# rs-anderson/explicit-alignment-for-vqa-tasks

Hardware: AMD Instinct MI355X
Metric: mapper_train_samples_per_sec (higher is better)
Workload: dtype bf16; 1 GPU; cfg2: CLIP ViT-B/32 -> GPT-2-large (774M), MLP mapper, prefix 10, CC-shaped synthetic batches; per-GPU batch 64, S=42; fwd+bwd+AdamW; random-init weights; global_batch=64, seq_len=42, parallelism=dp1

## Files before the change

### explicit-alignment-for-vqa-tasks_amd/_lib.py

```python
from __future__ import annotations

import ctypes as C
import os

_HERE = os.path.dirname(os.path.abspath(__file__))
LIB_PATH = os.path.join(_HERE, "csrc", "libeavqa_hip.so")

F32, BF16 = 0, 1
ACT = {"none": 0, "tanh": 1, "relu": 2, "gelu_new": 3, "quick_gelu": 4}

i32, i64, f32, ptr = C.c_int, C.c_int64, C.c_float, C.c_void_p

SIGNATURES = {
    "eavqa_abi_version": [],
    "eavqa_strerror": [i32],
    "eavqa_check_device": [],
    "eavqa_gemm": [i32, i32, i32, i32, i32, i32, ptr, i64, ptr, i64, ptr, i64, i32, f32, ptr, i32, ptr, ptr, i64, ptr, i64, ptr],
    "eavqa_layernorm_fwd": [i32, i32, i32, i32, ptr, i64, ptr, ptr, f32, ptr, i64, ptr, ptr, ptr],
    "eavqa_layernorm_bwd": [i32, i32, i32, i32, ptr, i64, ptr, i64, ptr, ptr, ptr, ptr, ptr, i64, ptr, ptr, ptr, i64, ptr],
    "eavqa_layernorm_fwd_fp8": [i32, i32, i32, ptr, i64, ptr, ptr, f32, ptr, i64, ptr, ptr, ptr, ptr],
    "eavqa_layernorm_bwd_fp8": [i32, i32, i32, ptr, i64, ptr, i64, ptr, ptr, ptr, ptr, ptr, i64, ptr, i64, ptr, ptr],
    "eavqa_attention_fwd": [i32, i32, i32, i32, i32, i32, ptr, i64, ptr, i64, ptr, i64, ptr, i64, i64, i64, ptr, i64, ptr, i32, f32, ptr, ptr],
    "eavqa_attention_decode": [i32, i32, i32, i32, i32, ptr, i64, ptr, i64, ptr, i64, i64, ptr, ptr, i64, ptr, i64, ptr, i64, f32, ptr],
    "eavqa_attention_decode_splitk": [i32, i32, i32, i32, i32, ptr, i32, ptr, ptr, i64, ptr, i64, i64, ptr, i64, ptr, i64, f32, ptr],
    "eavqa_attention_bwd": [i32, i32, i32, i32, i32, i32, ptr, i64, ptr, i64, ptr, i64, ptr, i64, ptr, i64,
                            ptr, i64, ptr, i64, ptr, i64, ptr, ptr, i32, f32, ptr, ptr, ptr],
    "eavqa_build_prefix_rows": [i32, i32, i32, ptr, ptr, i32, i32, i32, ptr, ptr, ptr, ptr],
    "eavqa_build_fewshot_rows": [i32, i32, i32, i32, i64, ptr, ptr, i32, ptr, ptr, ptr, ptr, ptr],
    "eavqa_build_row_plan": [i32, i32, i32, ptr, ptr, ptr, ptr, ptr, ptr, ptr, ptr, ptr, ptr],
    "eavqa_copy_rows": [i32, i32, i32, i32, ptr, i64, i64, ptr, i64, i64, i64, ptr],
    "eavqa_transpose": [i32, i32, i32, ptr, i64, ptr, i64, ptr],
    "eavqa_select_rows": [i32, ptr, i32, ptr, ptr, ptr, ptr],
    "eavqa_move_rows": [i32, i32, i32, i32, ptr, i64, ptr, ptr, i64, ptr],
    "eavqa_l2_normalize_rows": [i32, i32, ptr, i64, ptr],
    "eavqa_topk_rows": [i32, i32, ptr, i64, i32, ptr, ptr, ptr],
    "eavqa_gemm_splitk_plan": [i32, i32, i32],
    "eavqa_gemm_splitk": [i32, i32, i32, i32, ptr, i64, ptr, i64, ptr, i32, ptr],
    "eavqa_splitk_finish": [i32, i32, i32, ptr, i32, ptr, i32, ptr, i64, i32, i32, ptr, i64, ptr, i64, ptr, i64, ptr],
    "eavqa_layernorm_splitk": [i32, i32, i32, ptr, i64, ptr, i32, ptr, ptr, i64, ptr, ptr, f32, ptr, i64, ptr],
    "eavqa_gemm_fp8_splitk_plan": [i32, i32, i32],
    "eavqa_gemm_fp8_splitk": [i32, i32, i32, ptr, i64, ptr, ptr, i64, f32, ptr, i32, ptr],
    "eavqa_layernorm_splitk_fp8": [i32, i32, ptr, i64, ptr, i32, ptr, ptr, i64, ptr, ptr, f32, ptr, i64, ptr, ptr],
    "eavqa_rmsnorm_splitk": [i32, i32, i32, ptr, i64, ptr, i32, ptr, i64, ptr, f32, ptr, i64, ptr],
    "eavqa_splitk_finish_gated": [i32, i32, i32, ptr, i32, i32, ptr, i64, ptr],
    "eavqa_attention_decode_splitk_rel": [i32, i32, i32, i32, i32, ptr, i32, i32, ptr, i64, ptr, i64, i64, ptr, i64, ptr, i64, f32, ptr, i64, i32, ptr],
    "eavqa_colsum": [i32, i32, i32, ptr, i64, ptr, i32, ptr],
    "eavqa_embed_assemble": [i32, i32, i32, ptr, ptr, ptr, i64, ptr, i64, ptr, i64, ptr, i64, ptr],
# ... 103 lines not shown
```

### explicit-alignment-for-vqa-tasks_amd/csrc/gemm.hip

```cpp
#include "common.h"

namespace {

struct Knobs {
    int stagger;
    int ablate;
    bool disable_fast;
    int k64_mode;
    int big_mode;
    int deep;
    int shape_mode;
    int group_n;
    bool no_row_split;
    explicit Knobs(int k = 0) : stagger(k & 15), ablate((k >> 4) & 7), disable_fast(((k >> 7) & 1) != 0), k64_mode((k >> 8) & 63),
                                big_mode((k >> 14) & 3), deep((k >> 16) & 3), shape_mode((k >> 18) & 7), group_n((k >> 21) & 15),
                                no_row_split(((k >> 25) & 1) != 0) {}
};

struct GemmParamsBase {
    const void* A; const void* B; void* C;
    const float* bias; const void* aux_in; void* aux_out; const void* residual;
    const float* row_scale;
    int M, N, K;
    int64_t lda, ldb, ldc, ld_aux, ldr;
// ... 810 lines not shown
    if (m_cnt == 0 || local >= m_cnt * n_cnt) return false;
    const int GN = p.group_n;
    if (GN <= 0) {
        tm = m_begin + local % m_cnt;
        tn = n_begin + local / m_cnt;
        return true;
    }
    const int per_group = m_cnt * GN;
    const int g = local / per_group, r = local - g * per_group;
    const int gn = min(GN, n_cnt - g * GN);
    tm = m_begin + r / gn;
    tn = n_begin + g * GN + r % gn;
    return true;
}

template <bool LNX>
__global__ __launch_bounds__(1024) void gemm_bf16_big_kernel(typename KernArg<LNX>::type pk, int gx, int gy, int tiles_m, int tiles_n) {
    const GemmParams p = widen(pk);
    extern __shared__ __attribute__((aligned(16))) char smem[];
    int tm, tn;
    if (!big_tile(p, gx, gy, tiles_m, tiles_n, tm, tn)) return;
    const int m0 = tm * GBM, n0 = tn * GBN;
    const int tid = threadIdx.x, lane = tid & 63;
    const int wave = __builtin_amdgcn_readfirstlane(tid >> 6);
    const int wm = wave >> 2, wn = wave & 3;
    const bf16_t* A = reinterpret_cast<const bf16_t*>(p.A);
    const bf16_t* B = reinterpret_cast<const bf16_t*>(p.B);

    const bf16_t* asrc[2];
    const bf16_t* bsrc[2];
#pragma unroll
    for (int i = 0; i < 2; ++i) {
        const int c = tid + 1024 * i;
        const int row = c >> 3, pc = c & 7;
        asrc[i] = A + (int64_t)min(m0 + row, p.M - 1) * p.lda + (pc ^ (row & 7)) * 8;
        bsrc[i] = B + (int64_t)min(n0 + row, p.N - 1) * p.ldb + (pc ^ (row & 7)) * 8;
// ... 104 lines not shown
    if (rem == 0 || rem > 192 || M <= GBM) return 0;
    int gx, gy;
    const int tiles_n = (N + GBN - 1) / GBN;
    const int with = (big_grid((M + GBM - 1) / GBM, tiles_n, gx, gy) + 31) / 32, without = (big_grid(M / GBM, tiles_n, gx, gy) + 31) / 32;
    return without < with ? rem : 0;
}

bool use_big(const GemmParams& p, const Knobs& kn) {
    if (p.K % GBK) return false;
    if (kn.big_mode == 1) return false;
    if (kn.big_mode == 2) return true;
    const int tiles = ((p.M + GBM - 1) / GBM) * ((p.N + GBN - 1) / GBN);
    return tiles >= 144;
}


#include "gemm_k64.hip"

inline float k64_cost(const GemmParams& p, const K64Choice& c, float* multi_round_loop = nullptr) {
    const int tiles_m = (p.M + c.bm - 1) / c.bm, tiles_n = (p.N + c.bn - 1) / c.bn;
    const GridPlan g = plan_grid(tiles_m, tiles_n, c.bm, c.bn);
    const float rounds = float((g.per_xcd + 31) / 32);
    const float loop = rounds * c.rate * (c.bm + c.bn) * (p.K / 64);
    if (multi_round_loop) *multi_round_loop = rounds > 1.f ? loop : 0.f;
    return loop + rounds * 0.1f * c.bm * c.bn + 4500.f;
}

#include "gemm_fp8.hip"

template <int MF>
// ... 311 lines not shown
                             off(residual, r0, ldr, res_es), ldr, ln ? &ln2 : nullptr, stream, 0);
        };
        int bgx, bgy;
        const int big_rounds = (big_grid((M - big_rem + GBM - 1) / GBM, (N + GBN - 1) / GBN, bgx, bgy) + 31) / 32;
        const bool many_big_tiles = big_rounds >= 4 || (big_rounds >= 2 && (M + GBM - 1) / GBM > 96);
        if (a_kc && b_kc && !kn.disable_fast && (K % 64) == 0 && kn.k64_mode != 1 && kn.shape_mode == 0 && kn.big_mode == 0 && !many_big_tiles) {
            int pick = K64_AUTO[0];
            float best_loop = 0.f;
            float best = k64_cost(p, K64_SHAPES[pick], &best_loop);
            for (int i = 1; i < N_K64_AUTO; ++i) {
                float loop;
                const float c = k64_cost(p, K64_SHAPES[K64_AUTO[i]], &loop);
                if (c < best) { best = c; pick = K64_AUTO[i]; best_loop = loop; }
            }
            best += 0.35f * best_loop;
            const float big_cost = float(big_rounds) * (float(K / 64) * (big_rounds == 1 ? 1380.f : 1530.f) + 9000.f) + 3000.f + big_split_ns;
            if (M > 64 && big_cost < best) return run_big(p);
            return K64_SHAPES[pick].launch(p, s);
        }
        if (a_kc && b_kc && !kn.disable_fast && (K % FBK) == 0 && !ln) {
            if (kn.shape_mode >= 2 && kn.shape_mode < 7) return SHAPES[kn.shape_mode - 2].launch(p, s);
            const bool big_ok = (K % GBK) == 0 && kn.big_mode != 1;
            if (big_ok && kn.big_mode == 2) return run_big(p);
            float best = tile_cost(p, 128, 128, RATE_FAST);
            int pick = -1;
            if (big_ok && use_big(p, kn)) {
                GemmParams pf = p;
                pf.M = M - big_rem;
                best = fminf(best, tile_cost(pf, 256, 256, RATE_BIG) + big_split_ns);
                pick = -2;
// ... 5 lines not shown
                }
            if (pick >= 0) return SHAPES[pick].launch(p, s);
            if (pick == -2) return run_big(p);
            return launch_fast(p, s, kn);
        }
        if (a_kc && b_kc) return launch(gemm_bf16_kernel<true, true>, p, s);
        if (a_kc && !b_kc) return launch(gemm_bf16_kernel<true, false>, p, s);
        if (!a_kc && b_kc) return launch(gemm_bf16_kernel<false, true>, p, s);
        return launch(gemm_bf16_kernel<false, false>, p, s);
    }
    if (a_kc && b_kc) return launch(gemm_f32_kernel<true, true>, p, s);
    if (a_kc && !b_kc) return launch(gemm_f32_kernel<true, false>, p, s);
    if (!a_kc && b_kc) return launch(gemm_f32_kernel<false, true>, p, s);
    return launch(gemm_f32_kernel<false, false>, p, s);
}
}

extern "C" int eavqa_gemm_ex(int dtype, int a_kc, int b_kc, int M, int N, int K,
                             const void* A, int64_t lda, const void* B, int64_t ldb,
                             void* C, int64_t ldc, int out_flags, float alpha,
                             const float* bias, int act,
                             const void* aux_in, void* aux_out, int64_t ld_aux,
                             const void* residual, int64_t ldr, void* stream, int knobs) {
    return gemm_impl(dtype, a_kc, b_kc, M, N, K, A, lda, B, ldb, C, ldc, out_flags, alpha, bias, act, aux_in, aux_out, ld_aux, residual, ldr,
                     nullptr, stream, knobs);
}

extern "C" int eavqa_gemm_ln_ex(int dtype, int a_kc, int b_kc, int M, int N, int K,
                                const void* A, int64_t lda, const void* B, int64_t ldb,
                                void* C, int64_t ldc, int out_flags, float alpha,
// ... 92 lines not shown
```

### explicit-alignment-for-vqa-tasks_amd/csrc/gemm_k64.hip

```cpp
template <int N> __device__ __forceinline__ void wait_vm() { __builtin_amdgcn_s_waitcnt(vm_only(N)); }


template <int WM, int WN, int MF, int NF, int NST_, int LW_> struct K64SGeo {
    static constexpr int NST = NST_, LW = LW_;
    static constexpr int NC = WM * WN;
    static constexpr int NT = 64 * (NC + LW);
    static constexpr int TBM = 16 * MF * WM, TBN = 16 * NF * WN;
    static constexpr int PT = (TBM + TBN) / 8;
    static constexpr int P_LO = PT / LW, P_HI = (PT + LW - 1) / LW, N_HI = PT % LW;
    static constexpr int AOPER = TBM * 128, STAGE = (TBM + TBN) * 128, RING = NST * STAGE;
    static constexpr int PITCH = TBN + 4;
    static constexpr int SP = (16 * MF * WM * PITCH * 4 <= RING) ? WM : ((16 * MF * (WM / 2) * PITCH * 4 <= RING && WM >= 2) ? WM / 2 : 1);
    static constexpr int MFC = (16 * MF * PITCH * 4 <= RING) ? MF : MF / 2;
    static constexpr int PROWS = 16 * MFC * SP;
    static constexpr int TPR = TBN / 4;
    static constexpr int RPP = NT / TPR, NPASS = (PROWS + RPP - 1) / RPP;
    static_assert((TBM + TBN) % 8 == 0 && P_LO >= 1, "stage must cut into whole pieces, at least one per loader");
    static_assert(16 * MFC * PITCH * 4 <= RING && MF % MFC == 0 && (MFC == MF || SP == 1), "C staging pass must fit the ring");
    static_assert(WM % SP == 0 && RING <= 160 * 1024 && NT <= 1024, "geometry");
    static_assert(P_HI * (NST - 1) <= 63 && NST >= 2 && NST <= 6, "vmcnt field");
};

template <class G>
__device__ __forceinline__ void k64s_loader_role(const char* A, const char* B, int64_t lda_bytes, int64_t ldb_bytes, int M, int N, int m0,
// ... 187 lines not shown
}

struct K64Choice { int bm, bn, wg_per_cu; float rate; int (*launch)(const GemmParams&, hipStream_t); };
const K64Choice K64_SHAPES[] = {
    {128, 80, 2, 1.1f, launch_k64s<4, 1, 2, 5, 3, 2>},
    {128, 80, 2, 1.1f, launch_k64s<4, 1, 2, 5, 3, 4>},
    {128, 128, 2, 1.1f, launch_k64s<2, 2, 4, 4, 2, 4>},
    {256, 128, 1, 1.97f, launch_k64s<4, 2, 4, 4, 3, 4, true>},
    {256, 160, 1, 1.93f, launch_k64s<4, 2, 4, 5, 3, 4, true>},
    {128, 80, 1, 1.56f, launch_k64s<4, 1, 2, 5, 4, 2, true>},
    {128, 96, 1, 1.1f, launch_k64s<4, 1, 2, 6, 3, 2>},
    {256, 192, 1, 1.1f, launch_k64s<4, 2, 4, 6, 2, 4>},
    {256, 256, 1, 1.1f, launch_k64s<2, 4, 8, 4, 2, 4>},
    {128, 128, 1, 1.73f, launch_k64s<2, 2, 4, 4, 3, 2, true>},
    {128, 256, 1, 1.97f, launch_k64s<2, 4, 4, 4, 3, 4, true>},
};
constexpr int N_K64 = sizeof(K64_SHAPES) / sizeof(K64_SHAPES[0]);
constexpr int K64_AUTO[] = {5, 3, 4, 9, 10};
constexpr int N_K64_AUTO = sizeof(K64_AUTO) / sizeof(K64_AUTO[0]);
```

### explicit-alignment-for-vqa-tasks_amd/csrc/seq.hip

```cpp
#include "common.h"
#include <algorithm>

namespace {

__device__ __forceinline__ int wave_iscan(int v) {
    const int lane = threadIdx.x & 63;
#pragma unroll
    for (int o = 1; o < 64; o <<= 1) {
        const int t = __shfl_up(v, o, 64);
        if (lane >= o) v += t;
    }
    return v;
}

__device__ __forceinline__ void write_positions(const int* mrow, int S, int pos_mode, int32_t* pos_row) {
    const int lane = threadIdx.x & 63;
    int carry = 0;
    for (int s0 = 0; s0 < S; s0 += 64) {
        const int s = s0 + lane;
        const int mv = (s < S) ? mrow[s] : 0;
        const int inc = wave_iscan(mv) + carry;
        if (s < S) pos_row[s] = pos_mode == 0 ? s : (inc * mv - 1 + 2);
        carry = __shfl(inc, 63, 64);
    }
// ... 297 lines not shown
        const bool keep = lab >= 0;
        const unsigned long long bal = __ballot(keep);
        if (lane == 0) wave_n[wave] = __popcll(bal);
        __syncthreads();
        int off = base;
        for (int w = 0; w < wave; ++w) off += wave_n[w];
        const int pos = off + __popcll(bal & ((1ull << lane) - 1ull));
        if (keep && pos < cap) { sel_idx[pos] = r; sel_labels[pos] = lab; }
        __syncthreads();
        if (tid == 0) { int t = 0; for (int w = 0; w < 16; ++w) t += wave_n[w]; base += t; }
        __syncthreads();
    }
    if (tid == 0 && count) count[0] = base;
}

template <typename T, bool SCATTER>
__global__ __launch_bounds__(256) void move_rows_kernel(int cols, const T* __restrict__ src, int64_t lds, const int32_t* __restrict__ idx,
                                                        T* __restrict__ dst, int64_t ldd) {
    const int i = blockIdx.x, j = idx[i];
    const T* x = src + (int64_t)(SCATTER ? i : j) * lds;
    T* y = dst + (int64_t)(SCATTER ? j : i) * ldd;
    constexpr int V = 16 / sizeof(T);
    for (int c = threadIdx.x * V; c < cols; c += 256 * V) *reinterpret_cast<uint4*>(y + c) = *reinterpret_cast<const uint4*>(x + c);
}

__global__ void zero_kernel(int n, float* out) {
    const int i = blockIdx.x * blockDim.x + threadIdx.x;
    if (i < n) out[i] = 0.f;
}

// ... 19 lines not shown
        hipLaunchKernelGGL(copy_rows_kernel<float>, dim3(B * S), dim3(256), 0, s, S, cols, (const float*)src, lds, src_batch_rows,
                           (float*)dst, ldd, dst_batch_rows, dst_row0);
    else if (dtype == EAVQA_BF16)
        hipLaunchKernelGGL(copy_rows_kernel<bf16_t>, dim3(B * S), dim3(256), 0, s, S, cols, (const bf16_t*)src, lds, src_batch_rows,
                           (bf16_t*)dst, ldd, dst_batch_rows, dst_row0);
    else return EAVQA_E_DTYPE;
    EAVQA_LAUNCH_CHECK();
    return EAVQA_OK;
}

extern "C" int eavqa_select_rows(int M, const int64_t* row_labels, int capacity, int32_t* sel_idx, int64_t* sel_labels, int32_t* count,
                                 void* stream) {
    if (M <= 0 || capacity < 0 || !row_labels || !sel_idx || !sel_labels) return EAVQA_E_ARG;
    hipLaunchKernelGGL(select_rows_kernel, dim3(1), dim3(1024), 0, reinterpret_cast<hipStream_t>(stream), M, row_labels, capacity, sel_idx,
                       sel_labels, count);
    EAVQA_LAUNCH_CHECK();
    return EAVQA_OK;
}

extern "C" int eavqa_move_rows(int dtype, int scatter, int n, int cols, const void* src, int64_t ld_src, const int32_t* idx, void* dst,
                               int64_t ld_dst, void* stream) {
    if (n < 0 || cols <= 0 || !src || !idx || !dst) return EAVQA_E_ARG;
    if (n == 0) return EAVQA_OK;
    const int vec = dtype == EAVQA_BF16 ? 8 : 4;
    if (dtype != EAVQA_BF16 && dtype != EAVQA_F32) return EAVQA_E_DTYPE;
    if (cols % vec || ld_src % vec || ld_dst % vec || !eavqa_aligned16(src) || !eavqa_aligned16(dst)) return EAVQA_E_ALIGN;
    hipStream_t s = reinterpret_cast<hipStream_t>(stream);
    if (dtype == EAVQA_BF16) {
        if (scatter) hipLaunchKernelGGL((move_rows_kernel<bf16_t, true>), dim3(n), dim3(256), 0, s, cols, (const bf16_t*)src, ld_src, idx, (bf16_t*)dst, ld_dst);
        else hipLaunchKernelGGL((move_rows_kernel<bf16_t, false>), dim3(n), dim3(256), 0, s, cols, (const bf16_t*)src, ld_src, idx, (bf16_t*)dst, ld_dst);
// ... 211 lines not shown
```

### explicit-alignment-for-vqa-tasks_amd/models/lm.py

```python
from __future__ import annotations

import json
import math
import os
from dataclasses import dataclass
from typing import Dict, Optional

import torch

from .. import ops

Tensor = torch.Tensor


@dataclass
class LMConfig:
    arch: str
    n_layer: int
    n_head: int
    n_embd: int
    ffn: int
    vocab: int
    n_pos: int
    eps: float = 1e-5
# ... 186 lines not shown
                p = f"{pre}layers.{i}."
                L = _Layer()
                L.ln1_g, L.ln1_b = self._F(sd[p + "self_attn_layer_norm.weight"]), self._F(sd[p + "self_attn_layer_norm.bias"])
                L.w_qkv = self._T(torch.cat([sd[p + f"self_attn.{n}_proj.weight"] for n in "qkv"], dim=0))
                L.b_qkv = self._F(torch.cat([sd[p + f"self_attn.{n}_proj.bias"] for n in "qkv"], dim=0))
                L.w_o, L.b_o = self._T(sd[p + "self_attn.out_proj.weight"]), self._F(sd[p + "self_attn.out_proj.bias"])
                L.ln2_g, L.ln2_b = self._F(sd[p + "final_layer_norm.weight"]), self._F(sd[p + "final_layer_norm.bias"])
                L.w_fc1, L.b_fc1 = self._T(sd[p + "fc1.weight"]), self._F(sd[p + "fc1.bias"])
                L.w_fc2, L.b_fc2 = self._T(sd[p + "fc2.weight"]), self._F(sd[p + "fc2.bias"])
                L.w_qkv_t = L.w_o_t = L.w_fc1_t = L.w_fc2_t = None
                self.layers.append(L)
            self.lnf_g, self.lnf_b = self._F(sd[pre + "final_layer_norm.weight"]), self._F(sd[pre + "final_layer_norm.bias"])
            head = sd.get("lm_head.weight")
        self.head = self.wte if head is None or head.shape == self.wte.shape and _same(head, self.wte) else self._T(head)
        self.head_t = None
        self.head_q = None
        if self.weight_format == "fp8":
            for L in self.layers:
                for name in ("w_qkv", "w_o", "w_fc1", "w_fc2"):
                    setattr(L, name, Fp8Weight.quantize(getattr(L, name), self.device))
            self.head_q = Fp8Weight.quantize(self.head, self.device)

    @property
    def vocab(self) -> int:
        return self.wte.shape[0]

    @property
    def vpad(self) -> int:
        q = 128 if self.weight_format == "fp8" else 64
        return (self.vocab + q - 1) // q * q
# ... 61 lines not shown
        self.wte = self._T(weight)
        if tied:
            self.head = self.wte
        self._bwd_ready = False
        if self.weight_format == "fp8":
            self.head_q = Fp8Weight.quantize(self.head, self.device)

    def forward(self, prefix_rows: Optional[Tensor], src: Tensor, pos: Tensor, mask: Tensor, B: int, S: int, *,
                labels: Optional[Tensor] = None, save: bool = False, logits: str = "none", pack: bool = False,
                lengths=None, n_scored: Optional[int] = None):
        c, T = self.cfg, self.dtype
        E, H, hd = c.n_embd, c.n_head, c.head_dim
        scale = hd ** -0.5
        cu = flat = row_labels = None
        M = B * S
        if pack:
            cu, src_r, pos_r, row_labels, flat = ops.build_row_plan(mask, labels, src, pos, True)
            M = int(sum(lengths)) if lengths is not None else int(cu[-1].item())
            src, pos, flat = src_r[:M], pos_r[:M], flat[:M]
            row_labels = row_labels[:M] if labels is not None else None
            attn_mask = None
        else:
            attn_mask = mask
        x = ops.embed_assemble(src, pos, self.wte, prefix_rows, self.wpe)
        tape = [] if save else None
        fold = self.fold_layernorm and M > 64
        if fold:
            self._prepare_fold()
        n_slots = (E + 63) // 64
        f32 = dict(device=self.device, dtype=torch.float32)
        fuse_q = self.weight_format == "fp8" and self.fuse_quantizer

# ... 48 lines not shown
                tape.append((x, mean1, rstd1, qkv, ctx, lse, x1, mean2, rstd2, u))
            x = x2
        out = {"rows": M, "flat_index": flat}
        if logits == "last" and labels is None and not pack:
            xl = x.view(B, S, E)[:, -1]
            hf = ops.layernorm_fwd(xl, self.lnf_g, self.lnf_b, c.eps, T)
            out["logits"] = self._head(hf)
            return out
        if save:
            hf, meanf, rstdf = ops.layernorm_fwd(x, self.lnf_g, self.lnf_b, c.eps, T, save_stats=True)
        else:
            hf = ops.layernorm_fwd(x, self.lnf_g, self.lnf_b, c.eps, T)
        out["hidden"] = hf
        if labels is not None or logits == "all":
            sel = sel_count = None
            if pack and labels is not None and n_scored is not None and logits != "all" and 0 < n_scored < M:
                sel, ce_labels, sel_count = ops.select_rows(row_labels, int(n_scored))
                lg = self._head(ops.gather_rows(hf, sel))
            else:
                lg = self._head(hf)
                ce_labels = row_labels if pack else labels
            out["logits"], out["sel"] = lg, sel
            if labels is not None:
                loss, count, row_lse = ops.ce_fwd(lg, ce_labels, self.vocab)
                if sel_count is not None:
                    ops.guard_count(sel_count, int(n_scored), loss)
                out["loss"], out["count"] = loss, count
                if save:
                    out["tape"] = dict(layers=tape, x_last=x, meanf=meanf, rstdf=rstdf, logits=lg, labels=ce_labels, sel=sel,
                                       row_lse=row_lse, count=count, src=src, mask=attn_mask, cu=cu, B=B, S=S, M=M)
        return out

    def _head(self, hf: Tensor) -> Tensor:
        lg = torch.empty((hf.shape[0], self.vpad), device=self.device, dtype=torch.float32)
        if self.head_q is not None:
            linear(hf, self.head_q, out=lg[:, :self.vocab])
            return lg
        if hf.shape[0] <= 64 and hf.dtype == torch.bfloat16 and self.vocab % 4 == 0 and self.cfg.n_embd % 32 == 0:
            ops.splitk_finish(ops.gemm_splitk(hf, self.head[:self.vocab]), [lg[:, :self.vocab]])
        else:
            ops.gemm(hf, self.head, out=lg[:, :self.vocab])
        return lg

    def backward(self, tape: dict, gloss: Tensor, n_prefix_rows: int) -> Tensor:
        self._prepare_backward()
        c, T = self.cfg, self.dtype
        E, H, hd = c.n_embd, c.n_head, c.head_dim
        B, S, M = tape["B"], tape["S"], tape["M"]
        scale = hd ** -0.5
        mask, cu = tape["mask"], tape["cu"]
        lowp = T != torch.float32

        dlog = ops.ce_bwd(tape["logits"], tape["labels"], self.vocab, tape["row_lse"], tape["count"], gloss, T, self.vpad)
        dhf = linear(dlog, self.head_t)
        if tape.get("sel") is not None:
            dhf = ops.scatter_rows(dhf, tape["sel"], M)
        fuse_q = self.weight_format == "fp8" and self.fuse_quantizer
        if fuse_q:
            dxq = (torch.empty((M, E), device=self.device, dtype=torch.uint8), torch.empty(M, device=self.device, dtype=torch.float32))
            dxT = dxq

            def ln_bwd(xx, dy, g, mean, rstd, **kw):
                return ops.layernorm_bwd_fp8(xx, dy, g, mean, rstd, dxq[0], dxq[1], **kw)
        else:
            dxT = torch.empty((M, E), device=self.device, dtype=T) if lowp else None

            def ln_bwd(xx, dy, g, mean, rstd, **kw):
                return ops.layernorm_bwd(xx, dy, g, mean, rstd, lowp_out=dxT, **kw)
        dx = ln_bwd(tape["x_last"], dhf, self.lnf_g, tape["meanf"], tape["rstdf"])
        for L, (x, mean1, rstd1, qkv, ctx, lse, x1, mean2, rstd2, u) in zip(reversed(self.layers), reversed(tape["layers"])):
            du = linear(dxT if lowp else dx, L.w_fc2_t, act=c.act, aux_in=u)
# ... 18 lines not shown
```

### explicit-alignment-for-vqa-tasks_amd/ops.py

```python
from __future__ import annotations

import ctypes as C
from typing import Optional, Tuple

import torch

from . import _lib
from ._lib import ACT, BF16, F32, call

Tensor = torch.Tensor


F16 = 2


def dtype_id(dt: torch.dtype, stream: bool = False) -> int:
    if dt == torch.float32:
        return F32
    if dt == torch.bfloat16:
        return BF16
    if stream and dt == torch.float16:
        return F16
    raise _lib.EavqaError(f"unsupported storage dtype {dt}")


def _stream() -> int:
    return torch._C._cuda_getCurrentRawStream(torch._C._cuda_getDevice())


class KernelSelect:
    gemm = 0
    attention = 0
    decode_route = 0


def _p(t: Optional[Tensor]) -> Optional[int]:
    return None if t is None else t.data_ptr()


def _dev(t: Tensor) -> None:
    if not t.is_cuda:
        raise _lib.EavqaError("eavqa ops run on the GPU only (no CPU fallback): got a CPU tensor")


def _ld(t: Tensor) -> int:
    if t.stride(-1) != 1 and t.shape[-1] != 1:
        raise _lib.EavqaError("last dimension must be contiguous")
# ... 265 lines not shown

def build_row_plan(mask: Tensor, labels: Optional[Tensor], src: Tensor, pos: Tensor, pack: bool):
    _dev(mask)
    B, S = mask.shape
    dev = mask.device
    cu = torch.empty(B + 1, device=dev, dtype=torch.int32)
    src_r = torch.empty(B * S, device=dev, dtype=torch.int32)
    pos_r = torch.empty(B * S, device=dev, dtype=torch.int32)
    flat = torch.empty(B * S, device=dev, dtype=torch.int32)
    lab = torch.empty(B * S, device=dev, dtype=torch.int64)
    call("eavqa_build_row_plan", B, S, int(pack), _p(mask), _p(labels), _p(src), _p(pos), _p(cu), _p(src_r), _p(pos_r), _p(lab),
         _p(flat), _stream())
    return cu, src_r, pos_r, lab, flat


def _ce_dims(labels: Tensor):
    if labels.dim() == 2:
        return labels.shape[0], labels.shape[1], labels.shape[0] * labels.shape[1]
    return labels.shape[0], 0, labels.shape[0]


def ce_fwd(logits: Tensor, labels: Tensor, V: int):
    _dev(logits)
    B, S, rows = _ce_dims(labels)
    row_loss = torch.empty(rows, device=logits.device, dtype=torch.float32)
    row_lse = torch.empty(rows, device=logits.device, dtype=torch.float32)
    loss = torch.empty(1, device=logits.device, dtype=torch.float32)
    count = torch.empty(1, device=logits.device, dtype=torch.float32)
    call("eavqa_ce_fwd", B, S, V, _p(logits), _ld(logits), _p(labels), _p(row_loss), _p(row_lse), _p(loss), _p(count), _stream())
    return loss, count, row_lse
# ... 55 lines not shown
def copy_rows(src: Tensor, dst: Tensor, B: int, S: int, cols: int, src_batch_rows: int, dst_batch_rows: int, dst_row0: int) -> None:
    call("eavqa_copy_rows", dtype_id(src.dtype), B, S, cols, _p(src), _ld(src), src_batch_rows, _p(dst), _ld(dst),
         dst_batch_rows, dst_row0, _stream())


def colsum(x: Tensor, out: Tensor, accumulate: bool) -> None:
    rows, cols = x.shape
    call("eavqa_colsum", dtype_id(x.dtype), rows, cols, _p(x), _ld(x), _p(out), int(accumulate), _stream())


def transpose(x: Tensor, out: Optional[Tensor] = None) -> Tensor:
    rows, cols = x.shape
    y = out if out is not None else torch.empty((cols, rows), device=x.device, dtype=x.dtype)
    call("eavqa_transpose", dtype_id(x.dtype), rows, cols, _p(x), _ld(x), _p(y), _ld(y), _stream())
    return y


def gemm_splitk(a: Tensor, b: Tensor, ks: Optional[int] = None, unroll: int = 0, out: Optional[Tensor] = None) -> Tensor:
    M, K = a.shape
    N = b.shape[0]
    if ks is None:
        ks = int(_lib.load().eavqa_gemm_splitk_plan(M, N, K))
        if ks <= 0:
            raise _lib.EavqaError(f"eavqa_gemm_splitk: unsupported shape M={M} N={N} K={K}")
    part = out if out is not None else torch.empty((ks, M, N), device=a.device, dtype=torch.float32)
    if unroll:
        call("eavqa_gemm_splitk_ex", dtype_id(a.dtype), M, N, K, _p(a), _ld(a), _p(b), _ld(b), _p(part), ks, _stream(), unroll)
    else:
        call("eavqa_gemm_splitk", dtype_id(a.dtype), M, N, K, _p(a), _ld(a), _p(b), _ld(b), _p(part), ks, _stream())
    return part
# ... 206 lines not shown
```

### include/eavqa.h

```cpp
#ifndef EAVQA_H
#define EAVQA_H

#include <stdint.h>

#ifdef __cplusplus
extern "C" {
#endif
#pragma GCC visibility push(default)

#define EAVQA_ABI_VERSION 1

enum { EAVQA_F32 = 0, EAVQA_BF16 = 1,
       EAVQA_F16 = 2 };

enum { EAVQA_GEMM_OUT_F32 = 1, EAVQA_GEMM_RESIDUAL_LOWP = 2, EAVQA_GEMM_STREAM_F16 = 4 };
enum { EAVQA_ACT_NONE = 0, EAVQA_ACT_TANH = 1, EAVQA_ACT_RELU = 2, EAVQA_ACT_GELU_NEW = 3, EAVQA_ACT_QUICK_GELU = 4 };

enum {
    EAVQA_OK = 0,
    EAVQA_E_ARG = -1,
    EAVQA_E_ALIGN = -2,
    EAVQA_E_SHAPE = -3,
    EAVQA_E_DTYPE = -4,
    EAVQA_E_LAUNCH = -5,
// ... 61 lines not shown
                        const float* lse, float* delta, void* stream);

int eavqa_build_prefix_rows(int B, int L, int T, const int64_t* tokens, const int64_t* question_mask,
                            int pos_mode, int prefix_row_stride, int prefix_row_offset,
                            int32_t* src, int32_t* mask_out, int32_t* pos, void* stream);
int eavqa_build_fewshot_rows(int B, int T, int L, int n_img, int64_t special_token_id,
                             const int64_t* tokens, const int64_t* question_mask, int pos_mode,
                             int32_t* src, int32_t* mask_out, int32_t* pos, int32_t* status, void* stream);
int eavqa_build_row_plan(int B, int S, int pack, const int32_t* mask, const int64_t* labels, const int32_t* src,
                         const int32_t* pos, int32_t* cu_seqlens, int32_t* src_rows, int32_t* pos_rows,
                         int64_t* row_labels, int32_t* flat_index, void* stream);
int eavqa_copy_rows(int dtype, int B, int S, int cols, const void* src, int64_t lds, int64_t src_batch_rows,
                    void* dst, int64_t ldd, int64_t dst_batch_rows, int64_t dst_row0, void* stream);
int eavqa_select_rows(int M, const int64_t* row_labels, int capacity, int32_t* sel_idx, int64_t* sel_labels, int32_t* count,
                      void* stream);
int eavqa_move_rows(int dtype, int scatter, int n, int cols, const void* src, int64_t ld_src, const int32_t* idx, void* dst,
                    int64_t ld_dst, void* stream);
int eavqa_transpose(int dtype, int rows, int cols, const void* src, int64_t ld_src, void* dst, int64_t ld_dst, void* stream);
int eavqa_colsum(int dtype, int rows, int cols, const void* x, int64_t ldx, float* out, int accumulate, void* stream);
int eavqa_embed_assemble(int dtype, int rows, int E, const int32_t* src, const int32_t* pos,
                         const void* wte, int64_t ld_wte, const void* prefix_rows, int64_t ld_prefix,
                         const void* wpe, int64_t ld_wpe, float* x, int64_t ldx, void* stream);
int eavqa_embed_assemble_bwd(int dtype, int rows, int E, const int32_t* src, const float* dx, int64_t lddx,
                             void* dprefix, int64_t ld_dprefix, void* stream);

int eavqa_build_labels(int mode, int B, int T, int L, const int64_t* input_ids, int64_t pad_token_id,
                       int64_t bos_token_id, int64_t* labels_out, void* stream);

int eavqa_ce_fwd(int B, int S, int V, const float* logits, int64_t ld, const int64_t* labels,
                 float* row_loss, float* row_lse, float* loss, float* count, void* stream);
// ... 33 lines not shown
                               float eps, int B, int Sq, int row0, int S_max, float* x, const int32_t* key_mask, int64_t ld_mask,
                               void* workspace, int64_t workspace_bytes, void* stream);

typedef struct {
    const float* ln_sa; const void* w_qkv; const void* w_o;
    const float* ln_ca; const void* w_q_ca; const void* w_o_ca;
    const float* ln_ff; const void* w_i; const void* w_o_ff;
    void* k_cache; void* v_cache;
    const void* cross_kv;
} eavqa_t5_dec_layer_t;
int64_t eavqa_t5_decoder_step_workspace_bytes(int dtype, int B, int E, int inner, int F, int gated);
int eavqa_t5_decoder_step(int dtype, int n_layer, const eavqa_t5_dec_layer_t* layers, const float* ln_final, int E, int inner, int H,
                          int F, int gated, int act, float eps, int B, int t, int t_max, int S, float* x, void* out,
                          const int32_t* enc_mask, int64_t ld_mask, const float* rel_bias, int64_t rel_ld, int rel_zero,
                          void* workspace, int64_t workspace_bytes, void* stream);

int eavqa_gemm_splitk_plan(int M, int N, int K);
int eavqa_gemm_splitk(int dtype, int M, int N, int K, const void* A, int64_t lda, const void* B, int64_t ldb,
                      float* partials, int ks, void* stream);
int eavqa_splitk_finish(int dtype, int M, int N, const float* partials, int ks, const float* bias, int act,
                        const float* residual, int64_t ld_residual, int out_f32, int n_seg,
                        void* out0, int64_t ld0, void* out1, int64_t ld1, void* out2, int64_t ld2, void* stream);
int eavqa_layernorm_splitk(int dtype, int rows, int cols, const float* x_in, int64_t ldx, const float* partials, int ks,
                           const float* bias, float* x_out, int64_t ld_out, const float* gamma, const float* beta,
                           float eps, void* y, int64_t ldy, void* stream);

int eavqa_gemm_fp8_splitk_plan(int M, int N, int K);
int eavqa_gemm_fp8_splitk(int M, int N, int K, const void* A, int64_t lda, const float* a_row_scale, const void* B, int64_t ldb,
                          float b_scale, float* partials, int ks, void* stream);
int eavqa_layernorm_splitk_fp8(int rows, int cols, const float* x_in, int64_t ldx, const float* partials, int ks, const float* bias,
// ... 60 lines not shown
```

Baseline: 4785 samples/s.

## Add split-K head dgrad GEMM, deep-K tile shape, and fused scored row plan

Adds a deep-K split GEMM path that shards the vocab-length reduction of the LM-head input-gradient across workgroups. It writes per-slice fp32 partials and reduces them in a finish kernel that also scatters the selected rows, replacing the separate GEMM and scatter. The path only runs when `deepk_head_dgrad` is set, and that flag defaults to False. The change also adds an 80x80 K64 tile shape that the regular dispatcher considers for GEMMs with K of 16384 or more. It also fuses the row-plan build and scored-row selection into one kernel, saving a launch and a pass. The cost is extra workspace memory and a reduction pass, and the dispatcher's cost-model choices may shift.

```diff
diff --git a/explicit-alignment-for-vqa-tasks_amd/_lib.py b/explicit-alignment-for-vqa-tasks_amd/_lib.py
--- a/explicit-alignment-for-vqa-tasks_amd/_lib.py
+++ b/explicit-alignment-for-vqa-tasks_amd/_lib.py
@@ -31,6 +31,9 @@
     "eavqa_copy_rows": [i32, i32, i32, i32, ptr, i64, i64, ptr, i64, i64, i64, ptr],
     "eavqa_transpose": [i32, i32, i32, ptr, i64, ptr, i64, ptr],
     "eavqa_select_rows": [i32, ptr, i32, ptr, ptr, ptr, ptr],
+    "eavqa_build_scored_row_plan": [i32, i32, i32, ptr, ptr, ptr, ptr, ptr, ptr, ptr, ptr, ptr, i32, ptr, ptr, ptr, ptr],
+    "eavqa_gemm_deepk_plan": [i32, i32, i32, i64, C.POINTER(i64)],
+    "eavqa_gemm_deepk": [i32, i32, i32, i32, ptr, i64, ptr, i64, i32, ptr, i64, ptr, ptr, i32, i32, ptr, i64, ptr],
     "eavqa_move_rows": [i32, i32, i32, i32, ptr, i64, ptr, ptr, i64, ptr],
     "eavqa_l2_normalize_rows": [i32, i32, ptr, i64, ptr],
     "eavqa_topk_rows": [i32, i32, ptr, i64, i32, ptr, ptr, ptr],
diff --git a/explicit-alignment-for-vqa-tasks_amd/csrc/gemm.hip b/explicit-alignment-for-vqa-tasks_amd/csrc/gemm.hip
--- a/explicit-alignment-for-vqa-tasks_amd/csrc/gemm.hip
+++ b/explicit-alignment-for-vqa-tasks_amd/csrc/gemm.hip
@@ -848,12 +848,33 @@
     return true;
 }
 
-template <bool LNX>
+__device__ __forceinline__ bool deepk_unit(GemmParams& p, int slices, int tiles_m, int tiles_n, int& tm, int& tn) {
+    const int tiles = tiles_m * tiles_n, nwg = tiles * slices;
+    const int bid = blockIdx.x, q = nwg >> 3, r = nwg & 7, xcd = bid & 7, local = bid >> 3;
+    if (local >= q + (xcd < r ? 1 : 0)) return false;
+    const int unit = (xcd < r ? xcd * (q + 1) : r * (q + 1) + (xcd - r) * q) + local;
+    const int slice = unit / tiles, t = unit - slice * tiles;
+    tm = t % tiles_m;
+    tn = t / tiles_m;
+    const int nk = p.K >> 6, base = nk / slices, rem = nk % slices;
+    const int k0 = slice * base + min(slice, rem), cnt = base + (slice < rem ? 1 : 0);
+    p.A = reinterpret_cast<const bf16_t*>(p.A) + (int64_t)k0 * 64;
+    p.B = reinterpret_cast<const bf16_t*>(p.B) + (int64_t)k0 * 64;
+    p.K = cnt * 64;
+    p.C = reinterpret_cast<float*>(p.C) + (int64_t)slice * p.M * p.ldc;
+    return true;
+}
+
+template <bool LNX, bool DEEPK = false>
 __global__ __launch_bounds__(1024) void gemm_bf16_big_kernel(typename KernArg<LNX>::type pk, int gx, int gy, int tiles_m, int tiles_n) {
-    const GemmParams p = widen(pk);
+    GemmParams p = widen(pk);
     extern __shared__ __attribute__((aligned(16))) char smem[];
     int tm, tn;
-    if (!big_tile(p, gx, gy, tiles_m, tiles_n, tm, tn)) return;
+    if constexpr (DEEPK) {
+        if (!deepk_unit(p, gx, tiles_m, tiles_n, tm, tn)) return;
+    } else {
+        if (!big_tile(p, gx, gy, tiles_m, tiles_n, tm, tn)) return;
+    }
     const int m0 = tm * GBM, n0 = tn * GBN;
     const int tid = threadIdx.x, lane = tid & 63;
     const int wave = __builtin_amdgcn_readfirstlane(tid >> 6);
@@ -988,6 +1009,53 @@
     return tiles >= 144;
 }
 
+int launch_big_deepk(const GemmParams& p, int slices, hipStream_t stream) {
+    static std::atomic<bool> configured{false};
+    if (!configured.load(std::memory_order_acquire)) {
+        if (hipFuncSetAttribute(reinterpret_cast<const void*>(gemm_bf16_big_kernel<false, true>), hipFuncAttributeMaxDynamicSharedMemorySize,
+                                GLDS_BYTES) != hipSuccess)
+            return EAVQA_E_LAUNCH;
+        configured.store(true, std::memory_order_release);
+    }
+    const int tiles_m = (p.M + GBM - 1) / GBM, tiles_n = (p.N + GBN - 1) / GBN;
+    const int units = tiles_m * tiles_n * slices;
+    hipLaunchKernelGGL((gemm_bf16_big_kernel<false, true>), dim3((units + 7) / 8 * 8), dim3(1024), GLDS_BYTES, stream, p, slices, 0, tiles_m, tiles_n);
+    EAVQA_LAUNCH_CHECK();
+    return EAVQA_OK;
+}
+
+template <typename T>
+__global__ __launch_bounds__(256) void deepk_finish_kernel(int M, int N, const float* __restrict__ partials, int slices,
+                                                           const int32_t* __restrict__ sel, const int32_t* __restrict__ sel_count,
+                                                           T* __restrict__ out, int64_t ldc) {
+    const int r = blockIdx.x;
+    int i = r;
+    if (sel) {
+        const int n = sel_count ? min(M, max(sel_count[0], 0)) : M;
+        int lo = 0, hi = n;
+        while (lo < hi) {
+            const int mid = (lo + hi) >> 1;
+            if (sel[mid] < r) lo = mid + 1; else hi = mid;
+        }
+        i = (lo < n && sel[lo] == r) ? lo : -1;
+    }
+    T* y = out + (int64_t)r * ldc;
+    if (i < 0) {
+        for (int c = threadIdx.x * 4; c < N; c += 1024) elem<T>::st4(y + c, make_float4(0.f, 0.f, 0.f, 0.f));
+        return;
+    }
+    const int64_t slice_stride = (int64_t)M * N;
+    const float* x = partials + (int64_t)i * N;
+    for (int c = threadIdx.x * 4; c < N; c += 1024) {
+        float4 a = *reinterpret_cast<const float4*>(x + c);
+#pragma unroll 4
+        for (int s = 1; s < slices; ++s) {
+            const float4 t = *reinterpret_cast<const float4*>(x + s * slice_stride + c);
+            a.x += t.x; a.y += t.y; a.z += t.z; a.w += t.w;
+        }
+        elem<T>::st4(y + c, a);
+    }
+}
 
 #include "gemm_k64.hip"
 
@@ -1329,6 +1397,10 @@
                 if (c < best) { best = c; pick = K64_AUTO[i]; best_loop = loop; }
             }
             best += 0.35f * best_loop;
+            if (!ln && K >= K64_DEEP_MIN_K) {
+                const float c = k64_cost(p, K64_SHAPES[K64_DEEP]);
+                if (c < best) { best = c; pick = K64_DEEP; }
+            }
             const float big_cost = float(big_rounds) * (float(K / 64) * (big_rounds == 1 ? 1380.f : 1530.f) + 9000.f) + 3000.f + big_split_ns;
             if (M > 64 && big_cost < best) return run_big(p);
             return K64_SHAPES[pick].launch(p, s);
@@ -1364,6 +1436,76 @@
     if (!a_kc && b_kc) return launch(gemm_f32_kernel<false, true>, p, s);
     return launch(gemm_f32_kernel<false, false>, p, s);
 }
+
+float dispatch_cost(int M, int N, int K) {
+    GemmParams p;
+    p.M = M; p.N = N; p.K = K;
+    float best = 1e30f, best_loop = 0.f;
+    for (int i = 0; i < N_K64_AUTO; ++i) {
+        float loop;
+        const float c = k64_cost(p, K64_SHAPES[K64_AUTO[i]], &loop);
+        if (c < best) { best = c; best_loop = loop; }
+    }
+    best += 0.35f * best_loop;
+    if (K >= K64_DEEP_MIN_K) best = fminf(best, k64_cost(p, K64_SHAPES[K64_DEEP]));
+    int gx, gy;
+    const int big_rem = big_split_rows(M, N);
+    const int big_rounds = (big_grid((M - big_rem + GBM - 1) / GBM, (N + GBN - 1) / GBN, gx, gy) + 31) / 32;
+    const float big_cost = float(big_rounds) * (float(K / 64) * (big_rounds == 1 ? 1380.f : 1530.f) + 9000.f) + 3000.f + (big_rem ? 12000.f : 0.f);
+    return (M > 64 && big_cost < best) ? big_cost : best;
+}
+
+constexpr float DEEPK_KTILE_NS = 1450.f, DEEPK_FIXED_NS = 20000.f, DEEPK_RED_BYTES_PER_NS = 3500.f;
+constexpr int64_t DEEPK_MAX_WORKSPACE = int64_t(256) << 20;
+constexpr int DEEPK_MAX_SLICES = 32;
+}
+
+extern "C" int eavqa_gemm_deepk_plan(int M, int N, int K, int64_t max_workspace_bytes, int64_t* workspace_bytes) {
+    if (workspace_bytes) *workspace_bytes = 0;
+    if (M <= 64 || N <= 0 || K <= 0 || K % 64 || N % 4) return 0;
+    const int nk = K / 64, tiles = ((M + GBM - 1) / GBM) * ((N + GBN - 1) / GBN);
+    if (tiles >= 128 || nk < 32) return 0;
+    int best_s = 0;
+    float best = 0.8f * dispatch_cost(M, N, K);
+    for (int s = 2; s <= DEEPK_MAX_SLICES && s * 8 <= nk && tiles * s <= 256; ++s) {
+        const float ws = float(s) * float(M) * float(N) * 4.f;
+        const float c = float((nk + s - 1) / s) * DEEPK_KTILE_NS + DEEPK_FIXED_NS + ws / DEEPK_RED_BYTES_PER_NS;
+        if (c < best) { best = c; best_s = s; }
+    }
+    const int64_t ws = (int64_t)best_s * M * N * 4;
+    if (ws > (max_workspace_bytes > 0 ? max_workspace_bytes : DEEPK_MAX_WORKSPACE)) return 0;
+    if (workspace_bytes) *workspace_bytes = ws;
+    return best_s;
+}
+
+extern "C" int eavqa_gemm_deepk(int dtype, int M, int N, int K, const void* A, int64_t lda, const void* B, int64_t ldb, int slices,
+                                float* workspace, int64_t workspace_bytes, const int32_t* sel, const int32_t* sel_count, int out_rows,
+                                int out_f32, void* C, int64_t ldc, void* stream) {
+    if (dtype != EAVQA_BF16) return EAVQA_E_DTYPE;
+    if (!A || !B || !C || !workspace || M <= 0 || N <= 0 || K <= 0 || slices <= 0) return EAVQA_E_ARG;
+    if (K % 64 || N % 4 || slices > K / 64) return EAVQA_E_SHAPE;
+    if (lda % 8 || ldb % 8 || ldc % 4 || !eavqa_aligned16(A) || !eavqa_aligned16(B) || !eavqa_aligned16(workspace)) return EAVQA_E_ALIGN;
+    if ((reinterpret_cast<uintptr_t>(C) % (out_f32 ? 16 : 8)) != 0) return EAVQA_E_ALIGN;
+    if (lda < K || ldb < K || ldc < N) return EAVQA_E_ARG;
+    if (workspace_bytes < (int64_t)slices * M * N * 4) return EAVQA_E_ARG;
+    if (sel ? out_rows < M : out_rows != M) return EAVQA_E_ARG;
+    GemmParams p;
+    p.A = A; p.B = B; p.C = workspace; p.bias = nullptr; p.aux_in = nullptr; p.aux_out = nullptr; p.residual = nullptr; p.row_scale = nullptr; p.ablate = 0;
+    p.M = M; p.N = N; p.K = K; p.lda = lda; p.ldb = ldb; p.ldc = N; p.ld_aux = 0; p.ldr = 0;
+    p.act = EAVQA_ACT_NONE; p.out_f32 = 1; p.res_lowp = 0; p.out_f16 = 0; p.alpha = 1.0f;
+    p.group_n = 0;
+    p.tiles_m = (M + BM - 1) / BM;
+    p.tiles_n = (N + BN - 1) / BN;
+    p.vec_c = 1; p.vec_aux = 0; p.vec_res = 0; p.vec_bias = 0;
+    hipStream_t s = reinterpret_cast<hipStream_t>(stream);
+    const int rc = launch_big_deepk(p, slices, s);
+    if (rc) return rc;
+    if (out_f32)
+        hipLaunchKernelGGL(deepk_finish_kernel<float>, dim3(out_rows), dim3(256), 0, s, M, N, workspace, slices, sel, sel_count, reinterpret_cast<float*>(C), ldc);
+    else
+        hipLaunchKernelGGL(deepk_finish_kernel<bf16_t>, dim3(out_rows), dim3(256), 0, s, M, N, workspace, slices, sel, sel_count, reinterpret_cast<bf16_t*>(C), ldc);
+    EAVQA_LAUNCH_CHECK();
+    return EAVQA_OK;
 }
 
 extern "C" int eavqa_gemm_ex(int dtype, int a_kc, int b_kc, int M, int N, int K,
diff --git a/explicit-alignment-for-vqa-tasks_amd/csrc/gemm_k64.hip b/explicit-alignment-for-vqa-tasks_amd/csrc/gemm_k64.hip
--- a/explicit-alignment-for-vqa-tasks_amd/csrc/gemm_k64.hip
+++ b/explicit-alignment-for-vqa-tasks_amd/csrc/gemm_k64.hip
@@ -225,7 +225,9 @@
     {256, 256, 1, 1.1f, launch_k64s<2, 4, 8, 4, 2, 4>},
     {128, 128, 1, 1.73f, launch_k64s<2, 2, 4, 4, 3, 2, true>},
     {128, 256, 1, 1.97f, launch_k64s<2, 4, 4, 4, 3, 4, true>},
+    {80, 80, 1, 1.99f, launch_k64s<5, 1, 1, 5, 4, 2>},
 };
 constexpr int N_K64 = sizeof(K64_SHAPES) / sizeof(K64_SHAPES[0]);
 constexpr int K64_AUTO[] = {5, 3, 4, 9, 10};
 constexpr int N_K64_AUTO = sizeof(K64_AUTO) / sizeof(K64_AUTO[0]);
+constexpr int K64_DEEP = 11, K64_DEEP_MIN_K = 16384;
diff --git a/explicit-alignment-for-vqa-tasks_amd/csrc/seq.hip b/explicit-alignment-for-vqa-tasks_amd/csrc/seq.hip
--- a/explicit-alignment-for-vqa-tasks_amd/csrc/seq.hip
+++ b/explicit-alignment-for-vqa-tasks_amd/csrc/seq.hip
@@ -335,6 +335,74 @@
     if (tid == 0 && count) count[0] = base;
 }
 
+__global__ __launch_bounds__(1024) void row_plan_scored_kernel(int B, int S, int pack, const int32_t* __restrict__ mask,
+                                                               const int64_t* __restrict__ labels, const int32_t* __restrict__ src,
+                                                               const int32_t* __restrict__ pos, int32_t* __restrict__ cu,
+                                                               int32_t* __restrict__ src_p, int32_t* __restrict__ pos_p,
+                                                               int64_t* __restrict__ row_labels, int32_t* __restrict__ flat_index, int cap,
+                                                               int32_t* __restrict__ sel_idx, int64_t* __restrict__ sel_labels,
+                                                               int32_t* __restrict__ count) {
+    extern __shared__ int counts[];
+    int* lcounts = counts + B + 1;
+    const int tid = threadIdx.x, lane = tid & 63, wave = tid >> 6;
+    auto flags = [&](int b, int s, int& keep, int64_t& lab) {
+        const int64_t f = (int64_t)b * S + s;
+        keep = (s < S) && (!pack || mask[f] != 0) ? 1 : 0;
+        lab = (keep && s + 1 < S) ? labels[f + 1] : -100;
+    };
+    for (int b = wave; b < B; b += 16) {
+        int c = 0, l = 0;
+        for (int s0 = 0; s0 < S; s0 += 64) {
+            int keep;
+            int64_t lab;
+            flags(b, s0 + lane, keep, lab);
+            c += __popcll(__ballot(keep != 0));
+            l += __popcll(__ballot(lab >= 0));
+        }
+        if (lane == 0) { counts[b + 1] = c; lcounts[b + 1] = l; }
+    }
+    if (tid == 0) { counts[0] = 0; lcounts[0] = 0; }
+    __syncthreads();
+    if (wave == 0) {
+        int carry = 0, lcarry = 0;
+        for (int b0 = 0; b0 < B; b0 += 64) {
+            const int i = b0 + lane + 1;
+            const int inc = wave_iscan(i <= B ? counts[i] : 0) + carry;
+            const int linc = wave_iscan(i <= B ? lcounts[i] : 0) + lcarry;
+            if (i <= B) { counts[i] = inc; lcounts[i] = linc; }
+            carry = __shfl(inc, 63, 64);
+            lcarry = __shfl(linc, 63, 64);
+        }
+    }
+    __syncthreads();
+    for (int b = tid; b <= B; b += 1024) cu[b] = counts[b];
+    const int n_scored = lcounts[B];
+    if (tid == 0 && count) count[0] = n_scored;
+    for (int i = min(n_scored, cap) + tid; i < cap; i += 1024) { sel_idx[i] = 0; sel_labels[i] = -100; }
+    for (int b = wave; b < B; b += 16) {
+        int carry = counts[b], lcarry = lcounts[b];
+        for (int s0 = 0; s0 < S; s0 += 64) {
+            const int s = s0 + lane;
+            int keep;
+            int64_t lab;
+            flags(b, s, keep, lab);
+            const int inc = wave_iscan(keep) + carry;
+            const int linc = wave_iscan(lab >= 0 ? 1 : 0) + lcarry;
+            if (keep) {
+                const int r = inc - 1;
+                const int64_t f = (int64_t)b * S + s;
+                src_p[r] = src[f];
+                pos_p[r] = pos[f];
+                flat_index[r] = (int32_t)f;
+                row_labels[r] = lab;
+                if (lab >= 0 && linc - 1 < cap) { sel_idx[linc - 1] = r; sel_labels[linc - 1] = lab; }
+            }
+            carry = __shfl(inc, 63, 64);
+            lcarry = __shfl(linc, 63, 64);
+        }
+    }
+}
+
 template <typename T, bool SCATTER>
 __global__ __launch_bounds__(256) void move_rows_kernel(int cols, const T* __restrict__ src, int64_t lds, const int32_t* __restrict__ idx,
                                                         T* __restrict__ dst, int64_t ldd) {
@@ -384,6 +452,20 @@
     if (M <= 0 || capacity < 0 || !row_labels || !sel_idx || !sel_labels) return EAVQA_E_ARG;
     hipLaunchKernelGGL(select_rows_kernel, dim3(1), dim3(1024), 0, reinterpret_cast<hipStream_t>(stream), M, row_labels, capacity, sel_idx,
                        sel_labels, count);
+    EAVQA_LAUNCH_CHECK();
+    return EAVQA_OK;
+}
+
+extern "C" int eavqa_build_scored_row_plan(int B, int S, int pack, const int32_t* mask, const int64_t* labels, const int32_t* src,
+                                           const int32_t* pos, int32_t* cu_seqlens, int32_t* src_rows, int32_t* pos_rows,
+                                           int64_t* row_labels, int32_t* flat_index, int capacity, int32_t* sel_idx, int64_t* sel_labels,
+                                           int32_t* count, void* stream) {
+    if (B <= 0 || S <= 0 || capacity < 0 || !mask || !labels || !src || !pos || !cu_seqlens || !src_rows || !pos_rows || !row_labels ||
+        !flat_index || !sel_idx || !sel_labels)
+        return EAVQA_E_ARG;
+    if ((size_t)(B + 1) * 8 > 60 * 1024) return EAVQA_E_SHAPE;
+    hipLaunchKernelGGL(row_plan_scored_kernel, dim3(1), dim3(1024), (size_t)(B + 1) * 8, reinterpret_cast<hipStream_t>(stream), B, S, pack,
+                       mask, labels, src, pos, cu_seqlens, src_rows, pos_rows, row_labels, flat_index, capacity, sel_idx, sel_labels, count);
     EAVQA_LAUNCH_CHECK();
     return EAVQA_OK;
 }
diff --git a/explicit-alignment-for-vqa-tasks_amd/models/lm.py b/explicit-alignment-for-vqa-tasks_amd/models/lm.py
--- a/explicit-alignment-for-vqa-tasks_amd/models/lm.py
+++ b/explicit-alignment-for-vqa-tasks_amd/models/lm.py
@@ -224,6 +224,8 @@
             head = sd.get("lm_head.weight")
         self.head = self.wte if head is None or head.shape == self.wte.shape and _same(head, self.wte) else self._T(head)
         self.head_t = None
+        self._deepk_ws = None
+        self.deepk_head_dgrad = False
         self.head_q = None
         if self.weight_format == "fp8":
             for L in self.layers:
@@ -315,8 +317,12 @@
         scale = hd ** -0.5
         cu = flat = row_labels = None
         M = B * S
+        scored = None
+        if pack and labels is not None and n_scored is not None and logits != "all" and n_scored > 0:
+            cu, src_r, pos_r, row_labels, flat, *scored = ops.build_scored_row_plan(mask, labels, src, pos, True, int(n_scored))
+        elif pack:
+            cu, src_r, pos_r, row_labels, flat = ops.build_row_plan(mask, labels, src, pos, True)
         if pack:
-            cu, src_r, pos_r, row_labels, flat = ops.build_row_plan(mask, labels, src, pos, True)
             M = int(sum(lengths)) if lengths is not None else int(cu[-1].item())
             src, pos, flat = src_r[:M], pos_r[:M], flat[:M]
             row_labels = row_labels[:M] if labels is not None else None
@@ -395,8 +401,8 @@
         out["hidden"] = hf
         if labels is not None or logits == "all":
             sel = sel_count = None
-            if pack and labels is not None and n_scored is not None and logits != "all" and 0 < n_scored < M:
-                sel, ce_labels, sel_count = ops.select_rows(row_labels, int(n_scored))
+            if scored is not None and n_scored < M:
+                sel, ce_labels, sel_count = scored
                 lg = self._head(ops.gather_rows(hf, sel))
             else:
                 lg = self._head(hf)
@@ -408,7 +414,7 @@
                     ops.guard_count(sel_count, int(n_scored), loss)
                 out["loss"], out["count"] = loss, count
                 if save:
-                    out["tape"] = dict(layers=tape, x_last=x, meanf=meanf, rstdf=rstdf, logits=lg, labels=ce_labels, sel=sel,
+                    out["tape"] = dict(layers=tape, x_last=x, meanf=meanf, rstdf=rstdf, logits=lg, labels=ce_labels, sel=sel, sel_count=sel_count,
                                        row_lse=row_lse, count=count, src=src, mask=attn_mask, cu=cu, B=B, S=S, M=M)
         return out
 
@@ -433,9 +439,19 @@
         lowp = T != torch.float32
 
         dlog = ops.ce_bwd(tape["logits"], tape["labels"], self.vocab, tape["row_lse"], tape["count"], gloss, T, self.vpad)
-        dhf = linear(dlog, self.head_t)
-        if tape.get("sel") is not None:
-            dhf = ops.scatter_rows(dhf, tape["sel"], M)
+        sel = tape.get("sel")
+        slices = 0
+        if self.deepk_head_dgrad and isinstance(self.head_t, Tensor) and dlog.dtype == torch.bfloat16:
+            slices, ws_bytes = ops.gemm_deepk_plan(dlog.shape[0], E, self.vpad)
+        if slices:
+            if self._deepk_ws is None or self._deepk_ws.numel() < ws_bytes:
+                self._deepk_ws = torch.empty(ws_bytes, device=self.device, dtype=torch.uint8)
+            dhf = ops.gemm_deepk(dlog, self.head_t, slices, sel=sel, rows=M if sel is not None else None, sel_count=tape.get("sel_count"),
+                                 workspace=self._deepk_ws)
+        else:
+            dhf = linear(dlog, self.head_t)
+            if sel is not None:
+                dhf = ops.scatter_rows(dhf, sel, M)
         fuse_q = self.weight_format == "fp8" and self.fuse_quantizer
         if fuse_q:
             dxq = (torch.empty((M, E), device=self.device, dtype=torch.uint8), torch.empty(M, device=self.device, dtype=torch.float32))
diff --git a/explicit-alignment-for-vqa-tasks_amd/ops.py b/explicit-alignment-for-vqa-tasks_amd/ops.py
--- a/explicit-alignment-for-vqa-tasks_amd/ops.py
+++ b/explicit-alignment-for-vqa-tasks_amd/ops.py
@@ -31,6 +31,7 @@
 class KernelSelect:
     gemm = 0
     attention = 0
+    no_deepk = False
     decode_route = 0
 
 
@@ -326,6 +327,21 @@
     return cu, src_r, pos_r, lab, flat
 
 
+def build_scored_row_plan(mask: Tensor, labels: Tensor, src: Tensor, pos: Tensor, pack: bool, capacity: int):
+    _dev(mask)
+    B, S = mask.shape
+    dev = mask.device
+    sizes = [B + 1, B * S, B * S, B * S, capacity, 1]
+    pad4 = [(n + 3) // 4 * 4 for n in sizes]
+    i32 = torch.empty(sum(pad4), device=dev, dtype=torch.int32)
+    cu, src_r, pos_r, flat, idx, cnt = (t[:n] for t, n in zip(torch.split(i32, pad4), sizes))
+    i64 = torch.empty((B * S + 1) // 2 * 2 + capacity, device=dev, dtype=torch.int64)
+    lab, sel_lab = i64[:B * S], i64[(B * S + 1) // 2 * 2:]
+    call("eavqa_build_scored_row_plan", B, S, int(pack), _p(mask), _p(labels), _p(src), _p(pos), _p(cu), _p(src_r), _p(pos_r), _p(lab),
+         _p(flat), int(capacity), _p(idx), _p(sel_lab), _p(cnt), _stream())
+    return cu, src_r, pos_r, lab, flat, idx, sel_lab, cnt
+
+
 def _ce_dims(labels: Tensor):
     if labels.dim() == 2:
         return labels.shape[0], labels.shape[1], labels.shape[0] * labels.shape[1]
@@ -411,6 +427,33 @@
     y = out if out is not None else torch.empty((cols, rows), device=x.device, dtype=x.dtype)
     call("eavqa_transpose", dtype_id(x.dtype), rows, cols, _p(x), _ld(x), _p(y), _ld(y), _stream())
     return y
+
+
+def gemm_deepk_plan(M: int, N: int, K: int, max_workspace_bytes: int = 0) -> Tuple[int, int]:
+    if KernelSelect.no_deepk:
+        return 0, 0
+    ws = C.c_int64(0)
+    slices = int(_lib.load().eavqa_gemm_deepk_plan(int(M), int(N), int(K), int(max_workspace_bytes), C.byref(ws)))
+    return slices, int(ws.value)
+
+
+def gemm_deepk(a: Tensor, b: Tensor, slices: int, *, sel: Optional[Tensor] = None, rows: Optional[int] = None,
+               sel_count: Optional[Tensor] = None, out_dtype: Optional[torch.dtype] = None, workspace: Optional[Tensor] = None) -> Tensor:
+    _dev(a)
+    M, K = a.shape
+    N = b.shape[0]
+    if a.dtype != torch.bfloat16 or b.dtype != torch.bfloat16 or b.shape[1] != K:
+        raise _lib.EavqaError("gemm_deepk: bf16 operands [M,K] and [N,K]")
+    if sel is not None and (rows is None or sel.dtype != torch.int32 or sel.numel() != M):
+        raise _lib.EavqaError("gemm_deepk: sel must be int32 [M] and comes with the row count of the result")
+    out_dtype = out_dtype or a.dtype
+    need = slices * M * N * 4
+    if workspace is None:
+        workspace = torch.empty(need, device=a.device, dtype=torch.uint8)
+    out = torch.empty((rows if sel is not None else M, N), device=a.device, dtype=out_dtype)
+    call("eavqa_gemm_deepk", dtype_id(a.dtype), M, N, K, _p(a), _ld(a), _p(b), _ld(b), int(slices), _p(workspace), workspace.numel() * workspace.element_size(),
+         _p(sel), _p(sel_count) if sel is not None else None, out.shape[0], int(out_dtype == torch.float32), _p(out), _ld(out), _stream())
+    return out
 
 
 def gemm_splitk(a: Tensor, b: Tensor, ks: Optional[int] = None, unroll: int = 0, out: Optional[Tensor] = None) -> Tensor:
diff --git a/include/eavqa.h b/include/eavqa.h
--- a/include/eavqa.h
+++ b/include/eavqa.h
@@ -99,6 +99,10 @@
                     void* dst, int64_t ldd, int64_t dst_batch_rows, int64_t dst_row0, void* stream);
 int eavqa_select_rows(int M, const int64_t* row_labels, int capacity, int32_t* sel_idx, int64_t* sel_labels, int32_t* count,
                       void* stream);
+int eavqa_build_scored_row_plan(int B, int S, int pack, const int32_t* mask, const int64_t* labels, const int32_t* src,
+                                const int32_t* pos, int32_t* cu_seqlens, int32_t* src_rows, int32_t* pos_rows,
+                                int64_t* row_labels, int32_t* flat_index, int capacity, int32_t* sel_idx, int64_t* sel_labels,
+                                int32_t* count, void* stream);
 int eavqa_move_rows(int dtype, int scatter, int n, int cols, const void* src, int64_t ld_src, const int32_t* idx, void* dst,
                     int64_t ld_dst, void* stream);
 int eavqa_transpose(int dtype, int rows, int cols, const void* src, int64_t ld_src, void* dst, int64_t ld_dst, void* stream);
@@ -162,6 +166,11 @@
                           int F, int gated, int act, float eps, int B, int t, int t_max, int S, float* x, void* out,
                           const int32_t* enc_mask, int64_t ld_mask, const float* rel_bias, int64_t rel_ld, int rel_zero,
                           void* workspace, int64_t workspace_bytes, void* stream);
+
+int eavqa_gemm_deepk_plan(int M, int N, int K, int64_t max_workspace_bytes, int64_t* workspace_bytes);
+int eavqa_gemm_deepk(int dtype, int M, int N, int K, const void* A, int64_t lda, const void* B, int64_t ldb, int slices,
+                     float* workspace, int64_t workspace_bytes, const int32_t* sel, const int32_t* sel_count, int out_rows, int out_f32,
+                     void* C, int64_t ldc, void* stream);
 
 int eavqa_gemm_splitk_plan(int M, int N, int K);
 int eavqa_gemm_splitk(int dtype, int M, int N, int K, const void* A, int64_t lda, const void* B, int64_t ldb,
```

New measurement: 4803 samples/s, median of 3. Within noise of the previous version (+0.4%).
